# Contingencyy/CPUGPUPathtracing

Measured on AMD Instinct MI355X. Metric: Mrays/sec @ 1920x1080, 256 spp (dragon glTF stand-in), higher is better.
Workload: dtype f32

## Files before the change

### cpugpupathtracing_amd/csrc/device/wavefront_kernels.hip

```cpp
#include <hip/hip_runtime.h>

#include <algorithm>
#include <cstdint>
#include <cstdlib>
#include <new>

#include "cpugpupt_abi.h"
#include "device_scene.h"
#include "fast_div.h"
#include "rt_device.hpp"
#include "shade_device.hpp"
#include "trace_steps.hpp"
#include "accumulate.hpp"
#include "launch_common.h"

namespace cgpt {

using namespace dev;

hipStream_t CtxStream(cgpt_ctx* ctx);
void** CtxWavefrontSlot(cgpt_ctx* ctx);
hipEvent_t CtxStartEvent(cgpt_ctx* ctx);

extern __shared__ uint32_t lds_dyn[];

static constexpr uint32_t kMaxBands = 128;

struct WfDev {
    float4* A; float4* B; float4* C;
    float4* st_tp; float4* st_en;
    float4* px_hit;
    float4* brute;
    uint8_t* hit_flag;
    uint32_t* list_ext; uint32_t* list_sh;
    uint32_t* seg_ext; uint32_t* seg_sh;
    uint32_t* seg_count;
    uint32_t* seg_prefix;
    uint32_t n_bands;
    uint32_t band_magic;
    uint32_t* plan;
    uint32_t* stack_overflow;
    uint32_t cap;
    uint32_t n_paths;
    PathGrid g;
    uint32_t n_segs, seg_cap;
    uint32_t shade_chunk;
    uint32_t retire_misses;
    uint32_t rot_trace[2], rot_shade;
    unsigned long long* spec_tab;
    uint32_t spec_keys;
    uint32_t spec_epoch;
    uint32_t probe;
};

static constexpr uint32_t kChainShift = 10u, kChainMax = 0xFFFFu, kFollowerBit = 0x80000000u, kNoLeader = 0xFFFFFFFFu;
static constexpr uint32_t kSameRayBit = 0x40000000u;

__device__ __forceinline__ uint32_t elect_chain_leader(const WfDev& wf, uint32_t chain, uint32_t pid)
{
    const bool want = chain != 0u;
    uint32_t pixel = 0;
    if (want) { uint32_t sample_unused; path_split(wf.g, pid, sample_unused, pixel); }
    uint32_t src = lane_id();
    for (unsigned long long pend = __builtin_amdgcn_ballot_w64(want); pend != 0ull;) {
        const uint32_t f = (uint32_t)__builtin_ctzll(pend);
        const bool m = want && pixel == __builtin_amdgcn_readlane(pixel, f) && chain == __builtin_amdgcn_readlane(chain, f);
        if (m) src = f;
        pend &= ~__builtin_amdgcn_ballot_w64(m);
    }
    uint32_t leader = kNoLeader;
    if (want && src == lane_id()) {
        unsigned long long* const row = wf.spec_tab + (size_t)pixel * wf.spec_keys;
        const uint32_t tag = (wf.spec_epoch << 16) | chain;
        const unsigned long long mine = ((unsigned long long)pid << 32) | tag;
        for (uint32_t k = 0; k < wf.spec_keys; ++k) {
            unsigned long long cur = __hip_atomic_load(&row[k], __ATOMIC_RELAXED, __HIP_MEMORY_SCOPE_AGENT);
            while (((uint32_t)cur >> 16) != wf.spec_epoch) {
                const unsigned long long prev = atomicCAS(&row[k], cur, mine);
                cur = prev == cur ? mine : prev;
            }
            if ((uint32_t)cur == tag) { leader = (uint32_t)(cur >> 32); break; }
        }
    }
    return __shfl(leader, (int)src);
}


template <bool COUNT, bool FIRST, bool XFORM = false, bool TREE = false>
__global__ void __launch_bounds__(kTraceBlock, 1) wf_trace(const DevRenderArgs args, const WfDev wf, uint32_t batch_first, const TraceTune tune)
{
    constexpr bool first_round = FIRST;
    constexpr bool STEP = XFORM || TREE;
    const DevScene& sc = args.scene;
    DevCounters* const counters = args.counters;
    const TravCtx ctx = trav_setup(sc, lds_dyn, tune.top_records, wf.stack_overflow, gridDim.x * kTraceBlock, tune.lds_tris);
    lds_u32* const ring = ctx.ring;

    const uint32_t n_ext = first_round ? wf.g.n_pixels : wf.plan[0];
    const uint32_t n_sh = first_round ? 0u : wf.plan[1];
    const uint32_t blocks_ext = (n_ext + 63u) / 64u, n_blocks = blocks_ext + (n_sh + 63u) / 64u;
    const uint32_t n_waves = gridDim.x * (kTraceBlock / 64u);
    BlockWalk walk = first_block(blockIdx.x * (kTraceBlock / 64u) + __builtin_amdgcn_readfirstlane(threadIdx.x >> 6));
    uint32_t block = block_of(walk);
    const uint32_t rot = wf.rot_trace[first_round ? 1 : 0];
    uint32_t ring_count = 0;

    Trav r;
    r.d = mk(0.0f); r.rs = make_ray_slab(r.d, r.d); r.t = 0.0f;
    r.obj = kNoHit; r.tri = 0; r.depth = 0; r.cur_obj = 0; r.code = kIdle; r.sp = 0; r.fast_levels = kLdsStackLevels;
    if (XFORM) { r.wo = mk(0.0f); r.wd = mk(0.0f); trav_set_ray(r, r.wo, r.wd); }
    uint32_t slot_of_lane = 0;
    uint32_t wave_rays = 0;
    uint32_t wave_followers = 0;
    uint32_t wave_unwalked = 0;
    Counters cnt = { 0, 0, 0, 0, 0, 0 };

    auto finish_ray = [&]() {
        uint32_t slot = slot_of_lane;
        asm volatile("" : "+v"(slot));
        if (first_round) {
            float4 c; c.x = __uint_as_float(r.obj); c.y = __uint_as_float(r.tri); c.z = __uint_as_float(trav_depth(r)); c.w = r.t;
            st_stream(&wf.px_hit[slot], c);
        } else if (slot >= wf.cap) {
            if (r.obj == kNoHit) {
                const float4 pe = ld_stream(&wf.C[slot]);
                const uint32_t pid = slot - wf.cap;
                float4 en = ld_stream(&wf.st_en[pid]);
                en.x += pe.x; en.y += pe.y; en.z += pe.z;
                st_stream(&wf.st_en[pid], en);
            }
        } else {
            const bool hit = r.obj != kNoHit;
            if (wf.retire_misses) wf.hit_flag[slot] = hit ? (uint8_t)1 : (uint8_t)0;
            if (!wf.retire_misses || hit) {
                float4 c; c.x = __uint_as_float(r.obj); c.y = __uint_as_float(r.tri); c.z = __uint_as_float(trav_depth(r)); c.w = r.t;
                st_stream(&wf.C[slot], c);
            }
        }
        r.code = kIdle;
    };

    for (;;) {
        const unsigned long long need = __builtin_amdgcn_ballot_w64(r.code == kIdle);
        const uint32_t n_need = (uint32_t)__popcll(need);
        while (ring_count < n_need && block < n_blocks) {
            uint32_t s = 0; bool valid;
            if (block < blocks_ext) {
                const uint32_t i = block * 64u + lane_id();
                valid = i < n_ext;
                if (valid) s = first_round ? i : ld_stream(&wf.list_ext[i]);
            } else {
                const uint32_t i = (block - blocks_ext) * 64u + lane_id();
                valid = i < n_sh;
                if (valid) s = wf.cap + ld_stream(&wf.list_sh[i]);
            }
            const unsigned long long m = __builtin_amdgcn_ballot_w64(valid);
            if (valid) ring[ring_count + rank_in_mask(m)] = s;
            ring_count += (uint32_t)__popcll(m);
            next_block(walk, n_waves, rot);
            block = block_of(walk);
            __builtin_amdgcn_wave_barrier();
        }
        if (n_need && ring_count) {
            const uint32_t take = min(n_need, ring_count);
            const uint32_t rank = rank_in_mask(need);
            bool followed = false, unwalked = false;
            if (r.code == kIdle && rank < take) {
                const uint32_t slot = ring[ring_count - 1u - rank];
                slot_of_lane = slot;
                bool ok = true;
                V3 o, d; float t; uint32_t obj = kNoHit, tri = 0, depth = 0;
                if (first_round) {
                    Ray pr;
                    ok = pixel_ray(args, wf.g, slot, pr);
                    o = pr.o; d = pr.d; t = pr.t;
                } else {
                    const float4 a = ld_stream(&wf.A[slot]), b = ld_stream(&wf.B[slot]);
                    o = mk(a.x, a.y, a.z); t = a.w; d = mk(b.x, b.y, b.z);
                    if (!COUNT && slot < wf.cap && (__float_as_uint(b.w) & (kFollowerBit | kSameRayBit))) {
                        ok = false;
                        followed = (__float_as_uint(b.w) & kFollowerBit) != 0u; unwalked = !followed;
                        if (followed && wf.retire_misses) wf.hit_flag[slot] = 1;
                    } else if (slot < wf.cap && t != 1e34f) {
                        const float4 c = ld_stream(&wf.C[slot]);
                        obj = __float_as_uint(c.x); tri = __float_as_uint(c.y); depth = __float_as_uint(c.z);
                    }
                }
                if (ok) {
                    trav_start<XFORM, TREE>(ctx, r, o, d, t, obj, tri, depth);
                    if (!first_round && tune.shadow_any_hit != 0u && slot >= wf.cap) r.depth |= kAnyHitBit;
                    if (first_round) cnt.rays++;
                }
            }
            __builtin_amdgcn_wave_barrier();
            ring_count -= take;
            if (!first_round) wave_rays += take;
            if (!COUNT && !first_round) {
                wave_followers += (uint32_t)__popcll(__builtin_amdgcn_ballot_w64(followed));
                wave_unwalked += (uint32_t)__popcll(__builtin_amdgcn_ballot_w64(unwalked));
            }
        }
        if (__builtin_amdgcn_ballot_w64(r.code != kIdle) == 0ull && ring_count == 0u && block >= n_blocks) break;
        const bool can_refill = ring_count != 0u || block < n_blocks;

        for (;;) {
            const uint32_t n_inner = (uint32_t)__popcll(__builtin_amdgcn_ballot_w64(r.code < kStartObject));
            const uint32_t n_leaf = (uint32_t)__popcll(__builtin_amdgcn_ballot_w64((int32_t)r.code < 0));
            const uint32_t n_obj = (uint32_t)__popcll(__builtin_amdgcn_ballot_w64(r.code == kStartObject));
            const uint32_t n_busy = n_inner + n_leaf + n_obj;
            if (n_busy == 0u) break;
            if (can_refill && 64u - n_busy >= tune.refill_idle) break;
            const uint32_t w_obj = n_obj << tune.obj_shift;
            if (FIRST && tune.first_lean) {
                if (r.code < kStartObject || (int32_t)r.code < 0) lean_traverse<COUNT, !FIRST, STEP>(ctx, r, cnt);
                if (r.code == kStartObject && object_step<COUNT, !FIRST, XFORM, TREE>(ctx, r, cnt)) finish_ray();
                continue;
            }

            if (n_inner >= n_leaf && n_inner >= w_obj) {
                do {
                    if (r.code < kStartObject) inner_step<COUNT, STEP>(ctx, r, cnt);
                } while ((uint32_t)__popcll(__builtin_amdgcn_ballot_w64(r.code < kStartObject)) >= tune.inner_repeat);
            } else if (n_leaf >= w_obj) {
                do {
                    if ((int32_t)r.code < 0) leaf_step<COUNT, !FIRST, STEP>(ctx, r, cnt);
                } while ((uint32_t)__popcll(__builtin_amdgcn_ballot_w64((int32_t)r.code < 0)) >= tune.leaf_repeat);
            } else {
                do {
                    if (r.code == kStartObject && object_step<COUNT, !FIRST, XFORM, TREE>(ctx, r, cnt)) finish_ray();
                } while ((uint32_t)__popcll(__builtin_amdgcn_ballot_w64(r.code == kStartObject)) >= tune.obj_repeat);
            }
        }
    }

    const uint32_t per_ray = first_round ? wf.g.n_samples : 1u;
    if (first_round) wave_add_u64(&counters->traced_rays, cnt.rays, per_ray);
    else if (lane_id() == 0u && wave_rays) atomicAdd(&counters->traced_rays, (unsigned long long)wave_rays);
    if (!COUNT && !first_round && lane_id() == 0u && wave_followers) atomicAdd(&counters->chain_followers, (unsigned long long)wave_followers);
    if (!COUNT && !first_round && lane_id() == 0u && wave_unwalked) atomicAdd(&counters->retrace_unwalked, (unsigned long long)wave_unwalked);
    if (COUNT) {
        wave_add_u64(&counters->inner_steps, cnt.inner, per_ray);
        wave_add_u64(&counters->tri_tests, cnt.tris, per_ray);
        wave_add_u64(&counters->bvh_depth_sum, cnt.depth, per_ray);
    }
}

template <bool COUNT, bool FIRST, bool BRUTE = false, int LOBES = 0, bool RIS = false>
__global__ void __launch_bounds__(256, 1) wf_shade(const DevRenderArgs args, const WfDev wf, uint32_t batch_first)
{
    constexpr bool first_round = FIRST;
    constexpr bool kChains = !COUNT && !BRUTE;
    const DevScene& sc = args.scene;
    const uint32_t n_ext = first_round ? wf.n_paths : wf.plan[0];
    const uint32_t n_blocks = (n_ext + 63u) / 64u;
    const uint32_t n_waves = gridDim.x * 4u;
    const uint32_t wave = blockIdx.x * 4u + (threadIdx.x >> 6);
    uint32_t* const out_ext = wf.seg_ext + (size_t)wave * wf.seg_cap;
    uint32_t* const out_sh = wf.seg_sh + (size_t)wave * wf.seg_cap;
    uint32_t count_ext = 0, count_sh = 0;
    const bool banded = wf.n_bands > 1u;
    uint32_t cur_band = 0, band_start_ext = 0, band_start_sh = 0;
    Counters cnt = { 0, 0, 0, 0, 0, 0 };
    const bool probe = !COUNT && wf.probe != 0u;
    uint32_t wave_probed = 0;
    uint32_t wave_absorbed = 0;

    const uint32_t chunk = wf.shade_chunk;
    const uint32_t n_chunks = (n_blocks + chunk - 1u) / chunk;
    BlockWalk walk = first_block(wave);
    uint32_t ci = wave, block = ci * chunk, block_end = min((ci + 1u) * chunk, n_blocks);
    bool more = ci < n_chunks;
    auto advance = [&]() {
        if (++block >= block_end) {
            next_block(walk, n_waves, wf.rot_shade);
            ci = block_of(walk);
            more = ci < n_chunks;
            block = ci * chunk; block_end = min((ci + 1u) * chunk, n_blocks);
        }
    };
    __shared__ uint32_t s_queue[4][128];
    uint32_t* const queue = s_queue[threadIdx.x >> 6];
    uint32_t queued = 0;
    const bool hits_only = !first_round && wf.retire_misses != 0u;

    for (;;) {
        bool active = false;
        bool emit_ext = false, emit_sh = false;
        bool decided_sh = false, decided_ext = false;
        uint32_t pid = 0;
        uint32_t absorbed = 0;
        if (!hits_only) {
            if (!more) break;
            const uint32_t i = block * 64u + lane_id();
            active = i < n_ext;
            if (active) pid = first_round ? i : ld_stream(&wf.list_ext[i]);
            advance();
        } else {
            while (queued < 64u && more) {
                const uint32_t i = block * 64u + lane_id();
                uint32_t p = 0; bool hit = false;
                if (i < n_ext) { p = ld_stream(&wf.list_ext[i]); hit = wf.hit_flag[p] != 0; }
                const unsigned long long m = __builtin_amdgcn_ballot_w64(hit);
                if (hit) queue[queued + rank_in_mask(m)] = p;
                queued += (uint32_t)__popcll(m);
                advance();
            }
            if (queued == 0u) break;
            __builtin_amdgcn_wave_barrier();
            const uint32_t take = min(queued, 64u), rest = queued - take;
            active = lane_id() < take;
            if (active) pid = queue[lane_id()];
            const uint32_t moved = queue[64u + lane_id()];
            __builtin_amdgcn_wave_barrier();
            if (lane_id() < rest) queue[lane_id()] = moved;
            __builtin_amdgcn_wave_barrier();
            queued = rest;
        }
        if (active) {
            float4 c;
            Ray ray, shadow;
            PathState ps;
            bool is_pixel = true;
            bool brute_path = false;
            uint32_t chain = 0;
            bool followed = false;
            if (first_round) {
                uint32_t px = 0, pixel = 0;
                is_pixel = primary_ray(args, wf.g, pid, batch_first, ray, ps.rng, px, pixel);
                c = wf.px_hit[pixel];
                ps.throughput = mk(1.0f); ps.energy = mk(0.0f); ps.depth = 0; ps.is_specular = false;
                chain = 1u;
                if (BRUTE) brute_path = args.settings.render_mode == 1u || (args.settings.render_mode == 0u && px < args.width / 2u);
            } else {
                const float4 a = ld_stream(&wf.A[pid]), b = ld_stream(&wf.B[pid]);
                ray.o = mk(a.x, a.y, a.z); ray.d = mk(b.x, b.y, b.z);
                const float4 tp = ld_stream(&wf.st_tp[pid]);
                ps.throughput = mk(tp.x, tp.y, tp.z); ps.rng = __float_as_uint(tp.w);
                ps.energy = mk(0.0f);
                const uint32_t fl = __float_as_uint(b.w);
                ps.depth = fl & 0xFFu; ps.is_specular = (fl & 0x100u) != 0u;
                if (BRUTE) brute_path = (fl & 0x200u) != 0u;
                if (kChains) chain = (fl >> kChainShift) & kChainMax;
                if (kChains && (fl & kFollowerBit)) {
                    const uint32_t lead = __float_as_uint(a.w);
                    followed = true;
                    if (!wf.retire_misses || wf.hit_flag[lead]) c = ld_stream(&wf.C[lead]);
                    else { c.x = __uint_as_float(kNoHit); c.y = 0.0f; c.z = 0.0f; c.w = 0.0f; }
                } else c = ld_stream(&wf.C[pid]);
            }
            ray.t = c.w; ray.obj = __float_as_uint(c.x); ray.tri = __float_as_uint(c.y); ray.bvh_depth = __float_as_uint(c.z);
            shadow = ray;
            V3 pending = mk(0.0f);

            uint32_t flags = kBounceTerminate;
            if (BRUTE && brute_path) {
                if (is_pixel) {
                    const bool done = brute_level<COUNT, LOBES>(sc, args.settings, ray, ps.rng, ps.depth,
                        [&](uint32_t k, const BruteLevel& lv) {
                            float4* rec = wf.brute + ((size_t)k * wf.cap + pid) * 2u;
                            float4 r0, r1;
                            brute_pack(lv, r0, r1);
                            st_stream(&rec[0], r0); st_stream(&rec[1], r1);
                        },
                        [&](uint32_t k) { const float4* rec = wf.brute + ((size_t)k * wf.cap + pid) * 2u; return brute_unpack(ld_stream(&rec[0]), ld_stream(&rec[1])); },
                        ps.energy, cnt);
                    flags = done ? kBounceTerminate | kBounceBruteDone : 0u;
                }
            } else if (is_pixel) flags = shade_bounce<COUNT, LOBES, RIS>(sc, args.settings, ray, ps, shadow, pending, cnt);
            if (!COUNT) { absorbed = cnt.unwalked; cnt.unwalked = 0; }
            emit_ext = (flags & kBounceTerminate) == 0u;
            emit_sh = (flags & kBounceShadow) != 0u;
            if (kChains && emit_ext) {
                const uint32_t choice = (flags >> kBounceChainShift) & 3u;
                chain = choice != 0u && chain != 0u && chain <= (kChainMax - 2u) / 3u ? chain * 3u + choice - 1u : 0u;
            }
            bool connect = false;
            if (probe && !(BRUTE && brute_path)) {
                if (emit_sh) {
                    float t = shadow.t;
                    const uint32_t seen = probe_scene(sc, shadow.o, shadow.d, t);
                    decided_sh = seen != kProbeUndecided;
                    connect = seen == kProbeMiss;
                }
                if (emit_ext && !(kChains && chain != 0u) && ray.t == 1e34f) {
                    float t = ray.t;
                    decided_ext = probe_scene(sc, ray.o, ray.d, t) == kProbeMiss;
                }
                emit_sh = emit_sh && !decided_sh;
                emit_ext = emit_ext && !decided_ext;
            }

            const bool final_depth_needed = args.settings.debug_mode == 1u && !emit_ext;
            const bool own_energy = is_pixel && (first_round || (flags & (kBounceEnergy | kBounceBruteDone)) || final_depth_needed);
            if (own_energy || connect) {
                float4 en;
                if (first_round || (BRUTE && (flags & kBounceBruteDone))) { en.x = 0.0f; en.y = 0.0f; en.z = 0.0f; en.w = 0.0f; }
                else en = ld_stream(&wf.st_en[pid]);
                if (BRUTE && (flags & kBounceBruteDone)) { en.x = ps.energy.x; en.y = ps.energy.y; en.z = ps.energy.z; }
                if (flags & kBounceEnergy) { en.x += ps.energy.x; en.y += ps.energy.y; en.z += ps.energy.z; }
                if (own_energy) en.w = __uint_as_float(ps.depth & 0xFFu);
                if (connect) { en.x += pending.x; en.y += pending.y; en.z += pending.z; }
                st_stream(&wf.st_en[pid], en);
            }
            if (emit_ext) {
                float4 tpo;
                tpo.x = ps.throughput.x; tpo.y = ps.throughput.y; tpo.z = ps.throughput.z; tpo.w = __uint_as_float(ps.rng);
                st_stream(&wf.st_tp[pid], tpo);
                float4 na, nb;
                na.x = ray.o.x; na.y = ray.o.y; na.z = ray.o.z; na.w = ray.t;
                nb.x = ray.d.x; nb.y = ray.d.y; nb.z = ray.d.z;
                uint32_t fl = (ps.depth & 0xFFu) | (ps.is_specular ? 0x100u : 0u) | ((BRUTE && brute_path) ? 0x200u : 0u);
                if (((flags >> kBounceChainShift) & 3u) == kChainTir && !(BRUTE && brute_path)) fl |= kSameRayBit;
                if (kChains) {
                    fl |= chain << kChainShift;
                    if (wf.spec_tab) {
                        const uint32_t lead = elect_chain_leader(wf, chain, pid);
                        if (lead != kNoLeader && lead != pid) { na.w = __uint_as_float(lead); fl |= kFollowerBit; }
                    }
                }
                nb.w = __uint_as_float(fl);
                st_stream(&wf.A[pid], na); st_stream(&wf.B[pid], nb);
                if ((first_round || followed) && ray.t != 1e34f) st_stream(&wf.C[pid], c);
                if (first_round && !COUNT && wf.retire_misses && ray.t != 1e34f) wf.hit_flag[pid] = 1;
            }
            if (emit_sh) {
                const uint32_t ss = wf.cap + pid;
                float4 sa, sb, scc;
                sa.x = shadow.o.x; sa.y = shadow.o.y; sa.z = shadow.o.z; sa.w = shadow.t;
                sb.x = shadow.d.x; sb.y = shadow.d.y; sb.z = shadow.d.z; sb.w = 0.0f;
                scc.x = pending.x; scc.y = pending.y; scc.z = pending.z; scc.w = 0.0f;
                st_stream(&wf.A[ss], sa); st_stream(&wf.B[ss], sb); st_stream(&wf.C[ss], scc);
            }
        }
        const unsigned long long m_ext = __builtin_amdgcn_ballot_w64(emit_ext), m_sh = __builtin_amdgcn_ballot_w64(emit_sh);
        if (probe) wave_probed += (uint32_t)__popcll(__builtin_amdgcn_ballot_w64(decided_sh)) + (uint32_t)__popcll(__builtin_amdgcn_ballot_w64(decided_ext));
        if (!COUNT && __builtin_amdgcn_ballot_w64(absorbed != 0u) != 0ull)
            for (uint32_t b = 0; b < 8u; ++b) wave_absorbed += (uint32_t)__popcll(__builtin_amdgcn_ballot_w64((absorbed >> b) & 1u)) << b;
        if (banded) {
            const uint32_t band = min(wf.n_bands - 1u, __umulhi(pid, wf.band_magic));
            const bool emits = emit_ext | emit_sh;
            while (__builtin_amdgcn_ballot_w64(emits && band > cur_band) != 0ull) {
                const unsigned long long behind = __builtin_amdgcn_ballot_w64(band <= cur_band);
                const uint32_t end_ext = count_ext + (uint32_t)__popcll(m_ext & behind), end_sh = count_sh + (uint32_t)__popcll(m_sh & behind);
                if (lane_id() == 0u) {
                    wf.seg_count[cur_band * wf.n_segs + wave] = end_ext - band_start_ext;
                    wf.seg_count[(wf.n_bands + cur_band) * wf.n_segs + wave] = end_sh - band_start_sh;
                }
                band_start_ext = end_ext; band_start_sh = end_sh;
                ++cur_band;
            }
        }
        if (emit_ext) st_stream(&out_ext[count_ext + rank_in_mask(m_ext)], pid);
        if (emit_sh) st_stream(&out_sh[count_sh + rank_in_mask(m_sh)], pid);
        count_ext += (uint32_t)__popcll(m_ext);
        count_sh += (uint32_t)__popcll(m_sh);
    }
    if (banded) {
        if (lane_id() == 0u)
            for (uint32_t b = cur_band; b < wf.n_bands; ++b) {
                wf.seg_count[b * wf.n_segs + wave] = b == cur_band ? count_ext - band_start_ext : 0u;
                wf.seg_count[(wf.n_bands + b) * wf.n_segs + wave] = b == cur_band ? count_sh - band_start_sh : 0u;
            }
    } else if (lane_id() == 0) {
        wf.seg_count[wave] = count_ext; wf.seg_count[wf.n_segs + wave] = count_sh;
    }
    if (COUNT) wave_add_u64(&args.counters->closest_hits, cnt.hits);
    if (!COUNT && lane_id() == 0u && wave_probed) {
        atomicAdd(&args.counters->traced_rays, (unsigned long long)wave_probed);
        atomicAdd(&args.counters->probe_resolved, (unsigned long long)wave_probed);
    }
    if (!COUNT && lane_id() == 0u && wave_absorbed) {
        atomicAdd(&args.counters->traced_rays, (unsigned long long)wave_absorbed);
        atomicAdd(&args.counters->retrace_unwalked, (unsigned long long)wave_absorbed);
    }
}

__global__ void __launch_bounds__(256) wf_plan(const WfDev wf)
{
    __shared__ uint32_t partial[256];
    const uint32_t n = wf.n_segs;
    const uint32_t kk = blockIdx.x;
    const uint32_t* cnt = wf.seg_count + (size_t)kk * n;
    uint32_t* pre = wf.seg_prefix + (size_t)kk * n;
    const uint32_t per = (n + 255u) / 256u;
    const uint32_t begin = min(threadIdx.x * per, n), end = min(begin + per, n);
    uint32_t sum = 0;
    for (uint32_t i = begin; i < end; ++i) sum += cnt[i];
    partial[threadIdx.x] = sum;
    __syncthreads();
    for (uint32_t off = 1; off < 256u; off <<= 1) {
        const uint32_t v = threadIdx.x >= off ? partial[threadIdx.x - off] : 0u;
        __syncthreads();
        partial[threadIdx.x] += v;
        __syncthreads();
    }
    uint32_t run = partial[threadIdx.x] - sum;
    for (uint32_t i = begin; i < end; ++i) { pre[i] = run; run += cnt[i]; }
    if (threadIdx.x == 255u) {
        wf.plan[2u + kk] = partial[255];
        if (wf.n_bands == 1u) wf.plan[kk] = partial[255];
    }
}

__global__ void __launch_bounds__(256) wf_gather(const WfDev wf)
{
    typedef uint32_t u4a4 __attribute__((ext_vector_type(4), aligned(4)));
    if (wf.n_bands == 1u) {
        for (uint32_t s = blockIdx.x; s < 2u * wf.n_segs; s += gridDim.x) {
            const bool sh = s >= wf.n_segs;
            const uint32_t seg = sh ? s - wf.n_segs : s;
            const uint32_t n = wf.seg_count[s], base = wf.seg_prefix[s];
            const uint32_t* src = (sh ? wf.seg_sh : wf.seg_ext) + (size_t)seg * wf.seg_cap;
            uint32_t* dst = (sh ? wf.list_sh : wf.list_ext) + base;
            const uint32_t n4 = n & ~3u;
            for (uint32_t i = threadIdx.x * 4u; i < n4; i += blockDim.x * 4u) *reinterpret_cast<u4a4*>(dst + i) = *reinterpret_cast<const u4a4*>(src + i);
            if (threadIdx.x < n - n4) dst[n4 + threadIdx.x] = src[n4 + threadIdx.x];
        }
        return;
    }
    __shared__ uint32_t s_n[kMaxBands], s_dst[kMaxBands], s_src[kMaxBands];
    const uint32_t lane = threadIdx.x & 63u, wave_in_block = threadIdx.x >> 6;
    for (uint32_t s = blockIdx.x; s < 2u * wf.n_segs; s += gridDim.x) {
        const bool sh = s >= wf.n_segs;
        const uint32_t seg = sh ? s - wf.n_segs : s;
        const uint32_t* cnt = wf.seg_count + (sh ? wf.n_bands * wf.n_segs : 0u);
        const uint32_t* pre = wf.seg_prefix + (sh ? wf.n_bands * wf.n_segs : 0u);
        const uint32_t* band_total = wf.plan + 2u + (sh ? wf.n_bands : 0u);
        __syncthreads();
        if (threadIdx.x < wf.n_bands) {
            s_n[threadIdx.x] = cnt[threadIdx.x * wf.n_segs + seg];
            s_dst[threadIdx.x] = pre[threadIdx.x * wf.n_segs + seg];
            s_src[threadIdx.x] = band_total[threadIdx.x];
        }
        __syncthreads();
        if (threadIdx.x == 0u) {
            uint32_t off = 0, base = 0;
            for (uint32_t b = 0; b < wf.n_bands; ++b) {
                const uint32_t n = s_n[b], total = s_src[b];
                s_dst[b] += base; s_src[b] = off;
                off += n; base += total;
            }
            if (seg == 0u) wf.plan[sh ? 1 : 0] = base;
        }
        __syncthreads();
        const uint32_t* src = (sh ? wf.seg_sh : wf.seg_ext) + (size_t)seg * wf.seg_cap;
        uint32_t* const list = sh ? wf.list_sh : wf.list_ext;
        for (uint32_t b = wave_in_block; b < wf.n_bands; b += 4u) {
            const uint32_t n = s_n[b], n4 = n & ~3u;
            uint32_t* dst = list + s_dst[b];
            const uint32_t* run = src + s_src[b];
            for (uint32_t i = lane * 4u; i < n4; i += 256u) *reinterpret_cast<u4a4*>(dst + i) = *reinterpret_cast<const u4a4*>(run + i);
            if (lane < n - n4) dst[n4 + lane] = run[n4 + lane];
        }
    }
}

__global__ void __launch_bounds__(256) wf_accumulate(const DevRenderArgs args, const WfDev wf, uint32_t batch_first, uint32_t batch_n)
{
    accumulate_batch(args, wf.st_en, wf.g, batch_first, batch_n);
}

static constexpr uint32_t kMaxPools = 8;

struct WfTuning {
    uint32_t pools = 8;
    uint32_t batch = 0;
    uint32_t max_batch = 512;
    uint32_t pool_paths_mi = 512;
    uint32_t budget_gib = 96;
    uint32_t refill_idle = 16;
    uint32_t leaf_repeat = 4;
    uint32_t inner_repeat = 20;
    uint32_t obj_repeat = 1;
    uint32_t obj_shift = 0;
    uint32_t top_records = kLdsTopMax;
    uint32_t max_trace_blocks = 64;
    uint32_t shade_chunk = 4;
    uint32_t shade_chunk_banded = 32;
    uint32_t shadow_any_hit = 1;
    uint32_t lds_tris = 1;
    uint32_t first_lean = 1;
    uint32_t trace_events = 1;
    uint32_t path_order = 2;
    uint32_t retire_misses = 1;
    uint32_t bands_min_paths = 32u << 20;
    uint32_t bands = 32;
    uint32_t spec_dedupe = 1;
    uint32_t spec_keys = 8;
    uint32_t spec_epochs = 0xFFFF;
    uint32_t probe = 1;
    uint32_t probe_max_objects = 128;
};

static uint32_t Gcd(uint32_t a, uint32_t b) { while (b) { const uint32_t t = a % b; a = b; b = t; } return a; }
static uint32_t CoprimeRotation(uint32_t n_waves, uint32_t n_tiles)
{
    for (uint32_t rot = 0; rot < n_waves && rot < 4096u; ++rot)
        if (Gcd(n_waves + rot, std::max(1u, n_tiles)) == 1u) return rot;
    return 0u;
}

static decltype(&wf_trace<false, false>) const kTraceKernels[2][2][2] = {
    { { wf_trace<false, false>, wf_trace<false, true> }, { wf_trace<true, false>, wf_trace<true, true> } },
    { { wf_trace<false, false, true>, wf_trace<false, true, true> }, { wf_trace<true, false, true>, wf_trace<true, true, true> } },
};
static decltype(&wf_trace<false, false>) const kTraceTreeKernels[2][2][2] = {
    { { wf_trace<false, false, false, true>, wf_trace<false, true, false, true> }, { wf_trace<true, false, false, true>, wf_trace<true, true, false, true> } },
    { { wf_trace<false, false, true, true>, wf_trace<false, true, true, true> }, { wf_trace<true, false, true, true>, wf_trace<true, true, true, true> } },
};
#define CGPT_SHADE_LEVEL(G, R) \
    { { { wf_shade<false, false, false, G, R>, wf_shade<false, false, true, G, R> }, { wf_shade<false, true, false, G, R>, wf_shade<false, true, true, G, R> } }, \
      { { wf_shade<true, false, false, G, R>, wf_shade<true, false, true, G, R> }, { wf_shade<true, true, false, G, R>, wf_shade<true, true, true, G, R> } } }
static decltype(&wf_shade<false, false>) const kShadeKernels[2][kLobeLevels][2][2][2] = {
    { CGPT_SHADE_LEVEL(0, false), CGPT_SHADE_LEVEL(1, false), CGPT_SHADE_LEVEL(2, false), CGPT_SHADE_LEVEL(3, false), CGPT_SHADE_LEVEL(4, false) },
    { CGPT_SHADE_LEVEL(0, true), CGPT_SHADE_LEVEL(1, true), CGPT_SHADE_LEVEL(2, true), CGPT_SHADE_LEVEL(3, true), CGPT_SHADE_LEVEL(4, true) },
};
#undef CGPT_SHADE_LEVEL

struct WfSizes {
    uint32_t cap = 0, n_pixels = 0, n_segs = 0, seg_cap = 0;
    uint32_t overflow_words = 0;
    uint32_t brute_levels = 0;
    size_t spec = 0;
    bool Holds(const WfSizes& n) const
    {
        return cap >= n.cap && n_pixels >= n.n_pixels && n_segs >= n.n_segs && seg_cap >= n.seg_cap && overflow_words >= n.overflow_words &&
               brute_levels >= n.brute_levels && spec >= n.spec;
    }
};

template <typename F> static void ForEachBuffer(WfDev& d, const WfSizes& s, F&& f)
{
    const size_t slots = 2 * (size_t)s.cap * sizeof(float4), paths = s.cap, segs = (size_t)s.n_segs * s.seg_cap * sizeof(uint32_t);
    const size_t runs = 2 * (size_t)kMaxBands * s.n_segs * sizeof(uint32_t);
    f(d.A, slots); f(d.B, slots); f(d.C, slots);
    f(d.st_tp, paths * sizeof(float4)); f(d.st_en, paths * sizeof(float4)); f(d.hit_flag, paths);
    f(d.px_hit, (size_t)s.n_pixels * sizeof(float4));
    f(d.brute, (size_t)s.brute_levels * paths * 2u * sizeof(float4));
    f(d.list_ext, paths * sizeof(uint32_t)); f(d.list_sh, paths * sizeof(uint32_t));
    f(d.seg_ext, segs); f(d.seg_sh, segs);
    f(d.seg_count, runs); f(d.seg_prefix, runs);
    f(d.plan, (2 + 2 * (size_t)kMaxBands) * sizeof(uint32_t));
    f(d.stack_overflow, (size_t)s.overflow_words * sizeof(uint32_t));
    f(d.spec_tab, s.spec * sizeof(unsigned long long));
}

static size_t PoolBytes(const WfSizes& s)
{
    WfDev d{};
    size_t n = 0;
    ForEachBuffer(d, s, [&](auto*&, size_t bytes) { n += bytes; });
    return n;
}

struct WfHost {
    WfTuning tune;
    WfDev dev[kMaxPools] = {};
    hipStream_t streams[kMaxPools] = {};
    hipEvent_t acc_done[kMaxPools] = {};
    hipEvent_t begin = nullptr;
    WfSizes held;
    uint32_t held_pools = 0;
    uint32_t spec_epoch[kMaxPools] = {};
    uint32_t n_cus = 0;
    uint32_t trace_blocks_per_cu[2][2][2] = {}, shade_blocks_per_cu[2][kLobeLevels][2][2] = {};
    bool last_xform = false;
    uint32_t trace_tree_blocks_per_cu[2][2][2] = {};
    bool last_tree = false;
    size_t occupancy_lds = 0, tree_occupancy_lds = 0;
    EventPairs trace_ev;
    uint32_t trace_rounds = 0;
};

static void WfRelease(WfHost* h)
{
    for (uint32_t p = 0; p < kMaxPools; ++p) {
        ForEachBuffer(h->dev[p], h->held, [](auto*& ptr, size_t) { DevFree(ptr); });
        h->dev[p] = WfDev{};
    }
    h->held = WfSizes{}; h->held_pools = 0;
}

void WavefrontFree(void* state)
{
    if (!state) return;
    WfHost* h = static_cast<WfHost*>(state);
    WfRelease(h);
    for (uint32_t p = 0; p < kMaxPools; ++p) {
        if (h->streams[p]) (void)hipStreamDestroy(h->streams[p]);
        if (h->acc_done[p]) (void)hipEventDestroy(h->acc_done[p]);
    }
    if (h->begin) (void)hipEventDestroy(h->begin);
    FreeEvents(h->trace_ev);
    delete h;
}

uint32_t WavefrontTraceWavesPerSimd(void* state)
{
    if (!state) return 0;
    const WfHost* h = static_cast<const WfHost*>(state);
    return std::min(h->tune.max_trace_blocks, (h->last_tree ? h->trace_tree_blocks_per_cu : h->trace_blocks_per_cu)[h->last_xform][0][0]) * (kTraceBlock / 256u);
}

void WavefrontCollectTiming(void* state, double* trace_ms, uint32_t* trace_launches, double* round0_ms, uint32_t* round0_launches)
{
    *trace_ms = 0.0; *trace_launches = 0; *round0_ms = 0.0; *round0_launches = 0;
    if (!state) return;
    WfHost* h = static_cast<WfHost*>(state);
    ForEachPair(h->trace_ev, [&](uint32_t i, float ms) {
        *trace_ms += ms; *trace_launches += 1;
        if (h->trace_rounds && i % h->trace_rounds == 0u) { *round0_ms += ms; *round0_launches += 1; }
    });
}

static const Knob<WfTuning> kKnobs[] = {
    { "pools", &WfTuning::pools, 1, kMaxPools },           { "batch", &WfTuning::batch, 0, 4096 },
    { "max_batch", &WfTuning::max_batch, 1, 4096 },         { "pool_paths_mi", &WfTuning::pool_paths_mi, 1, 1024 },
    { "budget_gib", &WfTuning::budget_gib, 1, 256 },       { "refill", &WfTuning::refill_idle, 1, 64 },
    { "leaf_repeat", &WfTuning::leaf_repeat, 1, 65 },      { "inner_repeat", &WfTuning::inner_repeat, 1, 65 },
    { "obj_repeat", &WfTuning::obj_repeat, 1, 65 },        { "obj_shift", &WfTuning::obj_shift, 0, 6 },
    { "top_records", &WfTuning::top_records, 0, 4096 },     { "trace_blocks", &WfTuning::max_trace_blocks, 1, 64 },
    { "shade_chunk", &WfTuning::shade_chunk, 1, 256 },     { "shade_chunk_banded", &WfTuning::shade_chunk_banded, 1, 256 },
    { "shadow_any_hit", &WfTuning::shadow_any_hit, 0, 1 },     { "trace_events", &WfTuning::trace_events, 0, 1 },
    { "path_order", &WfTuning::path_order, 0, 2 },         { "retire_misses", &WfTuning::retire_misses, 0, 1 },
    { "lds_tris", &WfTuning::lds_tris, 0, 1 },             { "first_lean", &WfTuning::first_lean, 0, 1 },                     { "bands", &WfTuning::bands, 1, kMaxBands },             { "bands_min_paths", &WfTuning::bands_min_paths, 0, 0x7FFFFFFF },
    { "spec_dedupe", &WfTuning::spec_dedupe, 0, 1 },       { "spec_keys", &WfTuning::spec_keys, 1, 16 },
    { "spec_epochs", &WfTuning::spec_epochs, 1, 0xFFFF },   { "probe", &WfTuning::probe, 0, 1 },
    { "probe_max_objects", &WfTuning::probe_max_objects, 0, 4096 },
};

static WfHost* WfGetHost(cgpt_ctx* ctx)
{
    void** slot = CtxWavefrontSlot(ctx);
    if (*slot) return static_cast<WfHost*>(*slot);
    WfHost* fresh = new (std::nothrow) WfHost;
    if (!fresh) { CtxFail(ctx, CGPT_ERR_INVALID, "out of host memory"); return nullptr; }
    LoadKnobsFromEnv(kKnobs, "CGPT_WF_", fresh->tune);
    hipError_t e = hipEventCreateWithFlags(&fresh->begin, hipEventDisableTiming);
    for (uint32_t p = 0; p < kMaxPools && e == hipSuccess; ++p) {
        e = hipStreamCreateWithFlags(&fresh->streams[p], hipStreamNonBlocking);
        if (e == hipSuccess) e = hipEventCreateWithFlags(&fresh->acc_done[p], hipEventDisableTiming);
    }
    if (e != hipSuccess) {
        CtxFail(ctx, CGPT_ERR_HIP, "wavefront streams / events: %s", hipGetErrorString(e));
        WavefrontFree(fresh);
        return nullptr;
    }
    *slot = fresh;
    return fresh;
}

int WavefrontSetTuning(cgpt_ctx* ctx, const char* name, uint32_t value)
{
    WfHost* h = WfGetHost(ctx);
    return h ? SetKnob(ctx, FindKnob(kKnobs, name), h->tune, name, value) : CGPT_ERR_HIP;
}

int LaunchWavefront(cgpt_ctx* ctx, const DevRenderArgs& args_in, ShadeVariant v)
{
    hipStream_t stream = CtxStream(ctx);
    WfHost* h = WfGetHost(ctx);
    if (!h) return -1;
    const bool count = v.count;
    const uint32_t rows = args_in.n_rows;
    const uint32_t tiles_x = (args_in.width + 7u) / 8u, tiles_y = (rows + 7u) / 8u;
    const uint64_t n_pixels64 = (uint64_t)tiles_x * tiles_y * 64u;
    const uint32_t pool_paths = h->tune.pool_paths_mi << 20;
    if (n_pixels64 > pool_paths) { CtxFail(ctx, CGPT_ERR_UNSUPPORTED, "band of %llu pixels exceeds the wavefront pool", (unsigned long long)n_pixels64); return -1; }
    const uint32_t n_pixels = (uint32_t)n_pixels64;
    const uint32_t rounds = (uint32_t)args_in.settings.max_ray_depth + 2u;

    LAUNCH_TRY(QueryCuCount(h->n_cus));
    const uint32_t n_cus = h->n_cus;
    const uint32_t top_records = std::min(h->tune.top_records, args_in.scene.n_top_records);
    const size_t trace_lds = trace_lds_bytes(top_records);
    if (h->occupancy_lds != trace_lds) {
        static_assert(TableCount(kTraceKernels) == sizeof(h->trace_blocks_per_cu) / sizeof(uint32_t) && TableCount(kTraceTreeKernels) == sizeof(h->trace_tree_blocks_per_cu) / sizeof(uint32_t), "one occupancy entry per trace kernel");
        LAUNCH_TRY(QueryOccupancy(&kTraceKernels[0][0][0], &h->trace_blocks_per_cu[0][0][0], TableCount(kTraceKernels), kTraceBlock, trace_lds));
        uint32_t shade[2][kLobeLevels][2][2][2];
        static_assert(sizeof(shade) / sizeof(uint32_t) == TableCount(kShadeKernels), "one occupancy entry per shade kernel");
        LAUNCH_TRY(QueryOccupancy(&kShadeKernels[0][0][0][0][0], &shade[0][0][0][0][0], TableCount(kShadeKernels), 256, 0));
        for (int r = 0; r < 2; ++r)
            for (int g = 0; g < kLobeLevels; ++g)
                for (int c = 0; c < 2; ++c)
                    for (int b = 0; b < 2; ++b) h->shade_blocks_per_cu[r][g][c][b] = std::min(shade[r][g][c][0][b], shade[r][g][c][1][b]);
        h->occupancy_lds = trace_lds;
    }
    const dim3 block(256);
    const bool xform = HonoursTransforms((int)v.lobe_level);
    h->last_xform = xform;
    const bool tree = v.tree;
    h->last_tree = tree;
    if (tree && h->tree_occupancy_lds != trace_lds) {
        LAUNCH_TRY(QueryOccupancy(&kTraceTreeKernels[0][0][0], &h->trace_tree_blocks_per_cu[0][0][0], TableCount(kTraceTreeKernels), kTraceBlock, trace_lds));
        h->tree_occupancy_lds = trace_lds;
    }
    const uint32_t (&trace_blocks)[2][2][2] = tree ? h->trace_tree_blocks_per_cu : h->trace_blocks_per_cu;
    const auto& trace_kernels = tree ? kTraceTreeKernels : kTraceKernels;
    const dim3 trace_grid_first(n_cus * std::min(h->tune.max_trace_blocks, trace_blocks[xform][count][1]));
    const dim3 trace_grid_later(n_cus * std::min(h->tune.max_trace_blocks, trace_blocks[xform][count][0]));
    const bool brute = args_in.settings.render_mode != 2u;
    const uint32_t brute_levels = brute ? (uint32_t)args_in.settings.max_ray_depth + 1u : 0u;
    const uint32_t (&shade_blocks)[2][2] = h->shade_blocks_per_cu[v.ris][v.lobe_level];
    const dim3 shade_grid(n_cus * shade_blocks[count][brute]);
    const uint32_t n_segs = n_cus * std::max({ shade_blocks[0][0], shade_blocks[1][0], shade_blocks[0][1], shade_blocks[1][1] }) * 4u;
    const uint32_t min_shade_waves = n_cus * std::min({ shade_blocks[0][0], shade_blocks[1][0], shade_blocks[0][1], shade_blocks[1][1] }) * 4u;

    const uint32_t max_trace_threads = n_cus * std::max(*std::max_element(&h->trace_blocks_per_cu[0][0][0], &h->trace_blocks_per_cu[0][0][0] + TableCount(h->trace_blocks_per_cu)),
                                                        *std::max_element(&h->trace_tree_blocks_per_cu[0][0][0], &h->trace_tree_blocks_per_cu[0][0][0] + TableCount(h->trace_tree_blocks_per_cu))) * kTraceBlock;
    const uint32_t deep_levels = args_in.scene.stack_depth > kLdsStackLevels ? args_in.scene.stack_depth - kLdsStackLevels : 0u;
    const uint32_t overflow_words = std::max(1u, deep_levels * max_trace_threads);

    uint32_t shade_chunk = h->tune.shade_chunk;
    const bool chains = h->tune.spec_dedupe && !count && !brute;
    const size_t spec_entries = chains ? (size_t)n_pixels * h->tune.spec_keys : 0u;
    const size_t kBytesPerPath = 160 + 32 * (size_t)brute_levels;
    size_t free_b = 0, total_b = 0;
    LAUNCH_TRY(hipMemGetInfo(&free_b, &total_b));
    const size_t held_bytes = (size_t)h->held_pools * PoolBytes(h->held);
    const size_t budget = std::min<size_t>((size_t)h->tune.budget_gib << 30, (free_b + held_bytes) / 2);
    uint32_t batch = h->tune.batch;
    if (batch == 0) {
        batch = 1;
        while (batch < h->tune.max_batch && (uint64_t)n_pixels * batch * 2u <= (uint64_t)pool_paths) batch *= 2u;
    }
    batch = std::max(1u, std::min({ batch, std::max(1u, args_in.n_samples / 2u), args_in.n_samples, pool_paths / n_pixels }));
    WfSizes need;
    need.n_pixels = n_pixels; need.n_segs = n_segs; need.overflow_words = overflow_words; need.brute_levels = brute_levels; need.spec = spec_entries;
    uint32_t n_pools = 0, n_batches = 0;
    for (int attempt = 0;; ++attempt) {
        for (;;) {
            need.cap = n_pixels * batch;
            n_batches = (args_in.n_samples + batch - 1u) / batch;
            const uint32_t afford = (uint32_t)std::min<size_t>(kMaxPools, budget / ((size_t)need.cap * kBytesPerPath + spec_entries * sizeof(unsigned long long)));
            n_pools = std::max(1u, std::min({ h->tune.pools, n_batches, afford }));
            if (batch == 1u || (afford >= 1u && n_pools >= std::min({ 2u, n_batches, h->tune.pools }))) break;
            batch /= 2u;
        }
        const bool banded = h->tune.bands > 1u && need.cap >= h->tune.bands_min_paths;
        shade_chunk = banded ? h->tune.shade_chunk_banded : h->tune.shade_chunk;
        need.seg_cap = ((((need.cap + 63u) / 64u + shade_chunk - 1u) / shade_chunk + min_shade_waves - 1u) / min_shade_waves) * shade_chunk * 64u;
        if (h->held_pools >= n_pools && h->held.Holds(need)) break;
        LAUNCH_TRY(hipDeviceSynchronize());
        WfRelease(h);
        hipError_t err = hipSuccess;
        for (uint32_t p = 0; p < n_pools; ++p) {
            WfDev& d = h->dev[p];
            ForEachBuffer(d, need, [&](auto*& ptr, size_t bytes) { if (err == hipSuccess && bytes) err = DevAlloc((void**)&ptr, bytes); });
            if (err == hipSuccess && d.spec_tab) err = hipMemset(d.spec_tab, 0, need.spec * sizeof(unsigned long long));
            h->spec_epoch[p] = 0;
        }
        if (err == hipSuccess) { h->held = need; h->held_pools = n_pools; break; }
        (void)hipGetLastError();
        WfRelease(h);
        if (batch == 1u || attempt >= 8) { CtxFail(ctx, CGPT_ERR_HIP, "wavefront pools: %s", hipGetErrorString(err)); return -1; }
        batch /= 2u;
    }

    if (ReserveEvents(ctx, h->trace_ev, 2u * n_batches * rounds) != 0) return -1;
    h->trace_rounds = rounds;

    LAUNCH_TRY(hipEventRecord(CtxStartEvent(ctx), stream));
    LAUNCH_TRY(hipEventRecord(h->begin, stream));
    for (uint32_t p = 0; p < n_pools; ++p) LAUNCH_TRY(hipStreamWaitEvent(h->streams[p], h->begin, 0));

    int launches = 0;
    DevRenderArgs args = args_in;
    const TraceTune tt = { h->tune.refill_idle, h->tune.inner_repeat, h->tune.leaf_repeat, h->tune.obj_repeat, h->tune.obj_shift, top_records, h->tune.shadow_any_hit, h->tune.lds_tris, 0u, h->tune.first_lean };
    uint32_t k = 0;
    for (uint32_t done = 0; done < args_in.n_samples; done += batch, ++k) {
        const uint32_t p = k % n_pools;
        hipStream_t st = h->streams[p];
        const uint32_t bn = std::min(batch, args_in.n_samples - done);
        const uint32_t bfirst = args_in.first_sample + done;
        WfDev wf = h->dev[p];
        wf.cap = h->held.cap; wf.g.n_pixels = n_pixels; wf.n_paths = n_pixels * bn;
        wf.rot_trace[0] = CoprimeRotation(trace_grid_later.x * (kTraceBlock / 64u), tiles_x * tiles_y);
        wf.rot_trace[1] = CoprimeRotation(trace_grid_first.x * (kTraceBlock / 64u), tiles_x * tiles_y);
        wf.rot_shade = CoprimeRotation(shade_grid.x * 4u, std::max(1u, tiles_x * tiles_y / shade_chunk));
        wf.shade_chunk = shade_chunk;
        wf.g.tiles_x = tiles_x; wf.g.div_tiles_x = MakeFastDiv(tiles_x); wf.g.div_n_pixels = MakeFastDiv(n_pixels);
        wf.g.n_samples = bn; wf.g.div_samples = MakeFastDiv(bn); wf.g.order = h->tune.path_order; wf.n_segs = h->held.n_segs; wf.seg_cap = h->held.seg_cap;
        wf.n_bands = h->tune.bands > 1u && wf.n_paths >= h->tune.bands_min_paths ? h->tune.bands : 1u;
        if (wf.n_bands > 1u)
            wf.band_magic = (uint32_t)std::min<uint64_t>(0xFFFFFFFFull, (((uint64_t)wf.n_bands << 32) + wf.n_paths - 1u) / wf.n_paths);
        wf.retire_misses = h->tune.retire_misses && args_in.settings.debug_mode == 0u ? 1u : 0u;
        if (!chains) wf.spec_tab = nullptr;
        wf.spec_keys = h->tune.spec_keys;
        wf.probe = h->tune.probe && !count && !xform && !tree && args_in.settings.debug_mode == 0u && args_in.scene.n_objects <= h->tune.probe_max_objects ? 1u : 0u;
        if (k < n_pools) LAUNCH_TRY(hipMemsetAsync(wf.seg_count, 0, 2 * (size_t)kMaxBands * wf.n_segs * sizeof(uint32_t), st));
        for (uint32_t r = 0; r < rounds; ++r) {
            const bool first = r == 0u;
            if (h->tune.trace_events) LAUNCH_TRY(hipEventRecord(NextEvent(h->trace_ev), st));
            hipLaunchKernelGGL(trace_kernels[xform][count][first], first ? trace_grid_first : trace_grid_later, dim3(kTraceBlock), trace_lds, st, args, wf, bfirst, tt);
            if (h->tune.trace_events) LAUNCH_TRY(hipEventRecord(NextEvent(h->trace_ev), st));
            ++launches;
            if (r + 1u < rounds) {
                if (wf.spec_tab) {
                    if (++h->spec_epoch[p] > h->tune.spec_epochs) {
                        LAUNCH_TRY(hipMemsetAsync(wf.spec_tab, 0, h->held.spec * sizeof(unsigned long long), st));
                        h->spec_epoch[p] = 1u;
                    }
                    wf.spec_epoch = h->spec_epoch[p];
                }
                hipLaunchKernelGGL(kShadeKernels[v.ris][v.lobe_level][count][first][brute], shade_grid, block, 0, st, args, wf, bfirst);
                hipLaunchKernelGGL(wf_plan, dim3(2u * wf.n_bands), dim3(256), 0, st, wf);
                hipLaunchKernelGGL(wf_gather, dim3(std::min(2u * wf.n_segs, n_cus * 16u)), block, 0, st, wf);
                launches += 3;
            }
        }
        if (k > 0) LAUNCH_TRY(hipStreamWaitEvent(st, h->acc_done[(k - 1u) % n_pools], 0));
        hipLaunchKernelGGL(wf_accumulate, dim3(std::min((n_pixels + 255u) / 256u, n_cus * 8u)), block, 0, st, args, wf, bfirst, bn);
        ++launches;
        LAUNCH_TRY(hipEventRecord(h->acc_done[p], st));
        LAUNCH_TRY(hipGetLastError());
    }
    if (k > 0) LAUNCH_TRY(hipStreamWaitEvent(stream, h->acc_done[(k - 1u) % n_pools], 0));
    return launches;
}

}
```

Baseline: 21460.

## Read shade kernel args from kernarg segment, early-retire primary misses, cap shade blocks

The shade kernel now reads its parameters through a kernarg-segment pointer on demand instead of holding them in registers, and drops cached values such as chunk bounds and output pointers, to cut scalar/vector register pressure. First-round shading splits pixel lookup out, writes zero energy for primary misses and retires them before building the camera ray, and inlines seeding and camera-ray generation. A new tuning knob caps shade blocks per CU at 5 by default. The probe flag check is moved into per-path code, so the probe ballots now run even when probing is off, and the kernarg pointer trick depends on matching the parameter layout.

```diff
diff --git a/cpugpupathtracing_amd/csrc/device/wavefront_kernels.hip b/cpugpupathtracing_amd/csrc/device/wavefront_kernels.hip
--- a/cpugpupathtracing_amd/csrc/device/wavefront_kernels.hip
+++ b/cpugpupathtracing_amd/csrc/device/wavefront_kernels.hip
@@ -2,8 +2,10 @@
 
 #include <algorithm>
 #include <cstdint>
+#include <cstddef>
 #include <cstdlib>
 #include <new>
+#include <type_traits>
 
 #include "cpugpupt_abi.h"
 #include "device_scene.h"
@@ -245,43 +247,46 @@
     }
 }
 
+struct ShadeKernArgs { DevRenderArgs args; WfDev wf; uint32_t batch_first; };
+static_assert(alignof(DevRenderArgs) == 8 && alignof(WfDev) == 8 && sizeof(DevRenderArgs) % 8 == 0, "ShadeKernArgs mirrors the argument segment: every parameter at its natural alignment");
+__device__ __forceinline__ const ShadeKernArgs& shade_kernargs()
+{
+    const CGPT_UNIFORM ShadeKernArgs* p = (const CGPT_UNIFORM ShadeKernArgs*)__builtin_amdgcn_kernarg_segment_ptr();
+    asm volatile("" : "+s"(p));
+    return *(const ShadeKernArgs*)p;
+}
+
 template <bool COUNT, bool FIRST, bool BRUTE = false, int LOBES = 0, bool RIS = false>
-__global__ void __launch_bounds__(256, 1) wf_shade(const DevRenderArgs args, const WfDev wf, uint32_t batch_first)
+__global__ void __launch_bounds__(256, 1) wf_shade(const DevRenderArgs, const WfDev, uint32_t)
 {
     constexpr bool first_round = FIRST;
     constexpr bool kChains = !COUNT && !BRUTE;
-    const DevScene& sc = args.scene;
-    const uint32_t n_ext = first_round ? wf.n_paths : wf.plan[0];
+    uint32_t n_ext;
+    { const WfDev& wf = shade_kernargs().wf; n_ext = first_round ? wf.n_paths : wf.plan[0]; }
     const uint32_t n_blocks = (n_ext + 63u) / 64u;
     const uint32_t n_waves = gridDim.x * 4u;
-    const uint32_t wave = blockIdx.x * 4u + (threadIdx.x >> 6);
-    uint32_t* const out_ext = wf.seg_ext + (size_t)wave * wf.seg_cap;
-    uint32_t* const out_sh = wf.seg_sh + (size_t)wave * wf.seg_cap;
+    const uint32_t wave = blockIdx.x * 4u + __builtin_amdgcn_readfirstlane(threadIdx.x >> 6);
     uint32_t count_ext = 0, count_sh = 0;
-    const bool banded = wf.n_bands > 1u;
     uint32_t cur_band = 0, band_start_ext = 0, band_start_sh = 0;
     Counters cnt = { 0, 0, 0, 0, 0, 0 };
-    const bool probe = !COUNT && wf.probe != 0u;
     uint32_t wave_probed = 0;
     uint32_t wave_absorbed = 0;
 
-    const uint32_t chunk = wf.shade_chunk;
-    const uint32_t n_chunks = (n_blocks + chunk - 1u) / chunk;
     BlockWalk walk = first_block(wave);
-    uint32_t ci = wave, block = ci * chunk, block_end = min((ci + 1u) * chunk, n_blocks);
-    bool more = ci < n_chunks;
+    uint32_t block = wave * shade_kernargs().wf.shade_chunk;
+    auto more = [&]() { return block < n_blocks; };
     auto advance = [&]() {
-        if (++block >= block_end) {
+        const WfDev& wf = shade_kernargs().wf;
+        const uint32_t chunk = wf.shade_chunk;
+        if (++block >= min((block_of(walk) + 1u) * chunk, n_blocks)) {
             next_block(walk, n_waves, wf.rot_shade);
-            ci = block_of(walk);
-            more = ci < n_chunks;
-            block = ci * chunk; block_end = min((ci + 1u) * chunk, n_blocks);
+            block = block_of(walk) * chunk;
         }
     };
     __shared__ uint32_t s_queue[4][128];
     uint32_t* const queue = s_queue[threadIdx.x >> 6];
     uint32_t queued = 0;
-    const bool hits_only = !first_round && wf.retire_misses != 0u;
+    const bool hits_only = !first_round && shade_kernargs().wf.retire_misses != 0u;
 
     for (;;) {
         bool active = false;
@@ -290,13 +295,14 @@
         uint32_t pid = 0;
         uint32_t absorbed = 0;
         if (!hits_only) {
-            if (!more) break;
+            if (!more()) break;
             const uint32_t i = block * 64u + lane_id();
             active = i < n_ext;
-            if (active) pid = first_round ? i : ld_stream(&wf.list_ext[i]);
+            if (active) pid = first_round ? i : ld_stream(&shade_kernargs().wf.list_ext[i]);
             advance();
         } else {
-            while (queued < 64u && more) {
+            while (queued < 64u && more()) {
+                const WfDev& wf = shade_kernargs().wf;
                 const uint32_t i = block * 64u + lane_id();
                 uint32_t p = 0; bool hit = false;
                 if (i < n_ext) { p = ld_stream(&wf.list_ext[i]); hit = wf.hit_flag[p] != 0; }
@@ -316,22 +322,40 @@
             __builtin_amdgcn_wave_barrier();
             queued = rest;
         }
+        float4 c;
+        bool brute_path = false;
+        uint32_t sample = 0, px = 0, py = 0;
+        if (first_round && active) {
+            const ShadeKernArgs& ka = shade_kernargs();
+            const DevRenderArgs& args = ka.args;
+            uint32_t pixel, local_row;
+            path_split(ka.wf.g, pid, sample, pixel);
+            active = pixel_of_index(args, ka.wf.g, pixel, px, py, local_row);
+            if (active) {
+                c = ka.wf.px_hit[pixel];
+                if (BRUTE) brute_path = args.settings.render_mode == 1u || (args.settings.render_mode == 0u && px < args.width / 2u);
+                if (__float_as_uint(c.x) == kNoHit && args.settings.debug_mode != 2u && !(BRUTE && brute_path)) {
+                    float4 en; en.x = 0.0f; en.y = 0.0f; en.z = 0.0f; en.w = __uint_as_float(0u);
+                    st_stream(&ka.wf.st_en[pid], en);
+                    active = false;
+                }
+            }
+        }
         if (active) {
-            float4 c;
             Ray ray, shadow;
             PathState ps;
-            bool is_pixel = true;
-            bool brute_path = false;
+            constexpr bool is_pixel = true;
             uint32_t chain = 0;
             bool followed = false;
             if (first_round) {
-                uint32_t px = 0, pixel = 0;
-                is_pixel = primary_ray(args, wf.g, pid, batch_first, ray, ps.rng, px, pixel);
-                c = wf.px_hit[pixel];
+                const ShadeKernArgs& ka = shade_kernargs();
+                const DevRenderArgs& args = ka.args;
+                ps.rng = pcg_seed(py * args.width + px, ka.batch_first + sample, args.seed);
+                ray = camera_ray(args.camera, (float)px * (1.0f / (float)args.width), (float)py * (1.0f / (float)args.height));
                 ps.throughput = mk(1.0f); ps.energy = mk(0.0f); ps.depth = 0; ps.is_specular = false;
                 chain = 1u;
-                if (BRUTE) brute_path = args.settings.render_mode == 1u || (args.settings.render_mode == 0u && px < args.width / 2u);
             } else {
+                const WfDev& wf = shade_kernargs().wf;
                 const float4 a = ld_stream(&wf.A[pid]), b = ld_stream(&wf.B[pid]);
                 ray.o = mk(a.x, a.y, a.z); ray.d = mk(b.x, b.y, b.z);
                 const float4 tp = ld_stream(&wf.st_tp[pid]);
@@ -355,6 +379,10 @@
             uint32_t flags = kBounceTerminate;
             if (BRUTE && brute_path) {
                 if (is_pixel) {
+                    const ShadeKernArgs& ka = shade_kernargs();
+                    const DevScene& sc = ka.args.scene;
+                    const DevRenderArgs& args = ka.args;
+                    const WfDev& wf = ka.wf;
                     const bool done = brute_level<COUNT, LOBES>(sc, args.settings, ray, ps.rng, ps.depth,
                         [&](uint32_t k, const BruteLevel& lv) {
                             float4* rec = wf.brute + ((size_t)k * wf.cap + pid) * 2u;
@@ -366,7 +394,10 @@
                         ps.energy, cnt);
                     flags = done ? kBounceTerminate | kBounceBruteDone : 0u;
                 }
-            } else if (is_pixel) flags = shade_bounce<COUNT, LOBES, RIS>(sc, args.settings, ray, ps, shadow, pending, cnt);
+            } else if (is_pixel) {
+                const DevRenderArgs& args = shade_kernargs().args;
+                flags = shade_bounce<COUNT, LOBES, RIS>(args.scene, args.settings, ray, ps, shadow, pending, cnt);
+            }
             if (!COUNT) { absorbed = cnt.unwalked; cnt.unwalked = 0; }
             emit_ext = (flags & kBounceTerminate) == 0u;
             emit_sh = (flags & kBounceShadow) != 0u;
@@ -375,22 +406,23 @@
                 chain = choice != 0u && chain != 0u && chain <= (kChainMax - 2u) / 3u ? chain * 3u + choice - 1u : 0u;
             }
             bool connect = false;
-            if (probe && !(BRUTE && brute_path)) {
+            if (!COUNT && shade_kernargs().wf.probe != 0u && !(BRUTE && brute_path)) {
                 if (emit_sh) {
                     float t = shadow.t;
-                    const uint32_t seen = probe_scene(sc, shadow.o, shadow.d, t);
+                    const uint32_t seen = probe_scene(shade_kernargs().args.scene, shadow.o, shadow.d, t);
                     decided_sh = seen != kProbeUndecided;
                     connect = seen == kProbeMiss;
                 }
                 if (emit_ext && !(kChains && chain != 0u) && ray.t == 1e34f) {
                     float t = ray.t;
-                    decided_ext = probe_scene(sc, ray.o, ray.d, t) == kProbeMiss;
+                    decided_ext = probe_scene(shade_kernargs().args.scene, ray.o, ray.d, t) == kProbeMiss;
                 }
                 emit_sh = emit_sh && !decided_sh;
                 emit_ext = emit_ext && !decided_ext;
             }
 
-            const bool final_depth_needed = args.settings.debug_mode == 1u && !emit_ext;
+            const WfDev& wf = shade_kernargs().wf;
+            const bool final_depth_needed = shade_kernargs().args.settings.debug_mode == 1u && !emit_ext;
             const bool own_energy = is_pixel && (first_round || (flags & (kBounceEnergy | kBounceBruteDone)) || final_depth_needed);
             if (own_energy || connect) {
                 float4 en;
@@ -433,10 +465,11 @@
             }
         }
         const unsigned long long m_ext = __builtin_amdgcn_ballot_w64(emit_ext), m_sh = __builtin_amdgcn_ballot_w64(emit_sh);
-        if (probe) wave_probed += (uint32_t)__popcll(__builtin_amdgcn_ballot_w64(decided_sh)) + (uint32_t)__popcll(__builtin_amdgcn_ballot_w64(decided_ext));
+        if (!COUNT) wave_probed += (uint32_t)__popcll(__builtin_amdgcn_ballot_w64(decided_sh)) + (uint32_t)__popcll(__builtin_amdgcn_ballot_w64(decided_ext));
         if (!COUNT && __builtin_amdgcn_ballot_w64(absorbed != 0u) != 0ull)
             for (uint32_t b = 0; b < 8u; ++b) wave_absorbed += (uint32_t)__popcll(__builtin_amdgcn_ballot_w64((absorbed >> b) & 1u)) << b;
-        if (banded) {
+        const WfDev& wf = shade_kernargs().wf;
+        if (wf.n_bands > 1u) {
             const uint32_t band = min(wf.n_bands - 1u, __umulhi(pid, wf.band_magic));
             const bool emits = emit_ext | emit_sh;
             while (__builtin_amdgcn_ballot_w64(emits && band > cur_band) != 0ull) {
@@ -450,12 +483,15 @@
                 ++cur_band;
             }
         }
-        if (emit_ext) st_stream(&out_ext[count_ext + rank_in_mask(m_ext)], pid);
-        if (emit_sh) st_stream(&out_sh[count_sh + rank_in_mask(m_sh)], pid);
+        if (emit_ext) st_stream(&wf.seg_ext[(size_t)wave * wf.seg_cap + count_ext + rank_in_mask(m_ext)], pid);
+        if (emit_sh) st_stream(&wf.seg_sh[(size_t)wave * wf.seg_cap + count_sh + rank_in_mask(m_sh)], pid);
         count_ext += (uint32_t)__popcll(m_ext);
         count_sh += (uint32_t)__popcll(m_sh);
     }
-    if (banded) {
+    const ShadeKernArgs& ka = shade_kernargs();
+    const WfDev& wf = ka.wf;
+    const DevRenderArgs& args = ka.args;
+    if (wf.n_bands > 1u) {
         if (lane_id() == 0u)
             for (uint32_t b = cur_band; b < wf.n_bands; ++b) {
                 wf.seg_count[b * wf.n_segs + wave] = b == cur_band ? count_ext - band_start_ext : 0u;
@@ -474,6 +510,11 @@
         atomicAdd(&args.counters->retrace_unwalked, (unsigned long long)wave_absorbed);
     }
 }
+
+static_assert(std::is_same<decltype(&wf_shade<false, false>), void (*)(DevRenderArgs, WfDev, uint32_t)>::value &&
+              offsetof(ShadeKernArgs, args) == 0 && offsetof(ShadeKernArgs, wf) == sizeof(DevRenderArgs) &&
+              offsetof(ShadeKernArgs, batch_first) == sizeof(DevRenderArgs) + sizeof(WfDev),
+              "wf_shade reads its arguments through ShadeKernArgs: the struct and the parameter list change together");
 
 __global__ void __launch_bounds__(256) wf_plan(const WfDev wf)
 {
@@ -575,6 +616,7 @@
     uint32_t obj_shift = 0;
     uint32_t top_records = kLdsTopMax;
     uint32_t max_trace_blocks = 64;
+    uint32_t max_shade_blocks = 5;
     uint32_t shade_chunk = 4;
     uint32_t shade_chunk_banded = 32;
     uint32_t shadow_any_hit = 1;
@@ -720,6 +762,7 @@
     { "leaf_repeat", &WfTuning::leaf_repeat, 1, 65 },      { "inner_repeat", &WfTuning::inner_repeat, 1, 65 },
     { "obj_repeat", &WfTuning::obj_repeat, 1, 65 },        { "obj_shift", &WfTuning::obj_shift, 0, 6 },
     { "top_records", &WfTuning::top_records, 0, 4096 },     { "trace_blocks", &WfTuning::max_trace_blocks, 1, 64 },
+    { "shade_blocks", &WfTuning::max_shade_blocks, 1, 64 },
     { "shade_chunk", &WfTuning::shade_chunk, 1, 256 },     { "shade_chunk_banded", &WfTuning::shade_chunk_banded, 1, 256 },
     { "shadow_any_hit", &WfTuning::shadow_any_hit, 0, 1 },     { "trace_events", &WfTuning::trace_events, 0, 1 },
     { "path_order", &WfTuning::path_order, 0, 2 },         { "retire_misses", &WfTuning::retire_misses, 0, 1 },
@@ -801,7 +844,9 @@
     const dim3 trace_grid_later(n_cus * std::min(h->tune.max_trace_blocks, trace_blocks[xform][count][0]));
     const bool brute = args_in.settings.render_mode != 2u;
     const uint32_t brute_levels = brute ? (uint32_t)args_in.settings.max_ray_depth + 1u : 0u;
-    const uint32_t (&shade_blocks)[2][2] = h->shade_blocks_per_cu[v.ris][v.lobe_level];
+    uint32_t shade_blocks[2][2];
+    for (int c = 0; c < 2; ++c)
+        for (int b = 0; b < 2; ++b) shade_blocks[c][b] = std::min(h->tune.max_shade_blocks, h->shade_blocks_per_cu[v.ris][v.lobe_level][c][b]);
     const dim3 shade_grid(n_cus * shade_blocks[count][brute]);
     const uint32_t n_segs = n_cus * std::max({ shade_blocks[0][0], shade_blocks[1][0], shade_blocks[0][1], shade_blocks[1][1] }) * 4u;
     const uint32_t min_shade_waves = n_cus * std::min({ shade_blocks[0][0], shade_blocks[1][0], shade_blocks[0][1], shade_blocks[1][1] }) * 4u;
```

After: 21960 (median of 6 runs). 2.3% higher.
